# nreHieW/Eagle

Hardware: AMD Instinct MI355X
Metric: frames/sec end-to-end (detect+keypoint+homography) @1280x720 (higher is better)
Workload: dtype f32 (split: hi/lo binary16 pairs, 3 x fp16 MFMA per product, fp32 accumulate); detector (1.4 % of the FLOP): f32, exact v_mfma_f32_16x16x4_f32 chains

## Files before the change

eagle_amd/csrc/conv.hip:

```cpp
#include <algorithm>
#include <cmath>
#include <cstdlib>
#include <mutex>

#include "common.h"
#include "dmath.h"
#include "conv_internal.h"

namespace eagle {

static int f16_ps(int kc) { const int g = kc / 8; return kc * 2 + ((g % 2 == 0) ? 16 : 0); }
static int f16_ni(int ks, int kc) { return (ks * ks * (kc / 8) + 3) / 4; }

enum FormKind { GENERIC, WSTAT, ADIRECT };
enum StrideForm { S1, S2D, S2T, S1L };
enum WeightImage { W_F32, W_F16, W_F16_S2D, W_SPLIT, W_SPLIT_AD, W_SPLIT_S2D, W_SPLIT_M32 };
struct Form {
    int prec, variant, kind;
    int pw;
    int sform, rows, cols;
    int kc, nt, halo_bufs;
    int wimage;
    int grid_cap;
    ConvKernelGetter get;
};
static constexpr Form gen(int prec, int variant, int pw, int wimage, int kind = GENERIC) { return {prec, variant, kind, pw, S1, 0, 0, 0, 0, 0, wimage, 0, nullptr}; }
static constexpr Form ad(int prec, int variant, int sform, int rows, int cols, int nt, int halo_bufs, int wimage, ConvKernelGetter get, int grid_cap = 0)
{
    return {prec, variant, ADIRECT, 0, sform, rows, cols, prec == EAGLE_PREC_F16 ? 32 : 16, nt, halo_bufs, wimage, grid_cap, get};
}
static constexpr int F16 = EAGLE_PREC_F16, F32 = EAGLE_PREC_F32, F32S = EAGLE_PREC_F32S;
static constexpr Form g_forms[] = {
    gen(F32, 0, 4, W_F32), gen(F32, 3, 2, W_F32), gen(F32, 4, 1, W_F32),
    gen(F16, 0, 4, W_F16), gen(F16, 2, 4, W_F16), gen(F16, 3, 2, W_F16), gen(F16, 4, 1, W_F16), gen(F16, 6, 4, W_F16, WSTAT), gen(F16, 7, 2, W_F16, WSTAT),
    ad(F16, 8, S1, 4, 32, 12, 2, W_F16, conv_ad_kernel_s1_bn192), ad(F16, 9, S1, 8, 32, 6, 2, W_F16, conv_ad_kernel_s1_bn96),
    ad(F16, 10, S2D, 4, 32, 12, 2, W_F16_S2D, conv_ad_kernel_s2_bn192), ad(F16, 11, S2D, 8, 32, 6, 2, W_F16_S2D, conv_ad_kernel_s2_bn96),
    gen(F32S, 0, 4, W_SPLIT), gen(F32S, 3, 2, W_SPLIT), gen(F32S, 18, 6, W_SPLIT),
    ad(F32S, 8, S1, 4, 32, 12, 2, W_SPLIT_AD, conv_ad_split_kernel_bn192), ad(F32S, 9, S1, 8, 32, 6, 2, W_SPLIT_AD, conv_ad_split_kernel_bn96),
    ad(F32S, 10, S2D, 4, 32, 12, 2, W_SPLIT_S2D, conv_ad_split_kernel_s2_bn192), ad(F32S, 11, S2D, 8, 32, 6, 2, W_SPLIT_S2D, conv_ad_split_kernel_s2_bn96),
    ad(F32S, 12, S1, 8, 32, 3, 2, W_SPLIT_AD, conv_ad_split_kernel48), ad(F32S, 13, S1, 16, 32, 3, 1, W_SPLIT_AD, conv_ad_split_kernel48sb),
    ad(F32S, 19, S1, 16, 32, 3, 2, W_SPLIT_AD, conv_ad_split_kernel48ring, 256),
    ad(F32S, 14, S2T, 4, 32, 12, 1, W_SPLIT_AD, conv_ad_split_kernel_s2t_bn192), ad(F32S, 15, S2T, 4, 32, 6, 1, W_SPLIT_AD, conv_ad_split_kernel_s2t_bn96),
    ad(F32S, 21, S1, 4, 32, 12, 2, W_SPLIT_M32, conv_ad_split32_kernel_bn192), ad(F32S, 22, S1, 8, 32, 6, 2, W_SPLIT_M32, conv_ad_split32_kernel_bn96),
    ad(F32S, 23, S1, 2, 64, 12, 2, W_SPLIT_M32, conv_ad_split32_kernel_w64_bn192), ad(F32S, 24, S1, 4, 64, 6, 2, W_SPLIT_M32, conv_ad_split32_kernel_w64_bn96),
    ad(F32S, 27, S1L, 6, 30, 12, 2, W_SPLIT_M32, conv_ad_split32_kernel_lin30)};
static constexpr int LIN_PIXELS = 128;

static const Form* find_form(int precision, int variant)
{
    for (const Form& f : g_forms)
        if (f.prec == precision && f.variant == variant) return &f;
    return nullptr;
}
static const Form& form_of(int precision, const ConvConfig& c)
{
    const Form* f = find_form(precision, c.variant);
    if (!f) fail(EAGLE_E_NOKERNEL, "no conv kernel form: prec=%d variant=%d", precision, c.variant);
    return *f;
}
static int kind_of(int precision, const ConvConfig& c) { const Form* f = find_form(precision, c.variant); return f ? f->kind : -1; }

static size_t lds_bytes(int precision, const ConvConfig& c)
{
    const Form& f = form_of(precision, c);
    if (f.kind == ADIRECT) {
        int hpix, rec, strips;
        if (precision == EAGLE_PREC_F16) { hpix = f.sform == S2D ? (f.rows + 1) * 33 : (f.rows + 2) * 34; rec = 96; strips = 4 * 32 * 112; }
        else if (f.wimage == W_SPLIT_M32) { hpix = (f.rows + 2) * (f.cols + 2); rec = 80; strips = 4 * 32 * 128; }
        else { hpix = f.sform == S2T ? (2 * f.rows + 1) * 66 : (f.rows + 2) * 34; rec = 96; strips = 4 * 16 * 208; }
        const int slabs = ((hpix * rec + 1023) / 1024 + 3) / 4 * 4;
        return (size_t)f.halo_bufs * slabs * 1024 + strips;
    }
    const int th = 4 * f.pw / c.wx, tw = 16 * c.wx;
    const int hw = (tw - 1) * c.stride + c.ks, hh = (th - 1) * c.stride + c.ks;
    const int bn = c.nt * 16;
    if (precision == EAGLE_PREC_F16) {
        const size_t operands = (size_t)f16_ni(c.ks, c.kc) * 4 * bn * 16 + (size_t)hh * hw * f16_ps(c.kc);
        const size_t strips = (size_t)4 * f.pw * 16 * (bn * 2 + 16);
        return f.kind == WSTAT ? operands + strips + 16 : std::max(operands + 16, strips);
    }
    if (precision == EAGLE_PREC_F32S) {
        const size_t operands = (size_t)f16_ni(c.ks, c.kc) * 2 * 4 * bn * 16 + (size_t)hh * hw * f16_ps(2 * c.kc);
        const size_t strips = (size_t)4 * f.pw * 16 * (bn * 4 + 16);
        return std::max(operands + 16, strips);
    }
    return (size_t)c.ks * c.ks * (c.kc / 4) * 4 * bn * 4 + (size_t)hh * hw * (c.kc + 1) * 4;
}

size_t conv_lds_bytes(int precision, const ConvConfig& c) { return lds_bytes(precision, c); }
void conv_tile_shape(int precision, const ConvConfig& c, int* th, int* tw)
{
    const Form& f = form_of(precision, c);
    *th = f.kind == ADIRECT ? f.rows : 4 * f.pw / c.wx; *tw = f.kind == ADIRECT ? f.cols : 16 * c.wx;
}

int conv_tiles_per_frame(int precision, const ConvConfig& c, int ho, int wo)
{
    int th, tw;
    conv_tile_shape(precision, c, &th, &tw);
    if (form_of(precision, c).sform == S1L) return (ho * wo + LIN_PIXELS - 1) / LIN_PIXELS;
    return ((wo + tw - 1) / tw) * ((ho + th - 1) / th);
}

static const Inst* generic_inst(int precision, const ConvConfig& c)
{
    for (auto part : {conv_inst_part0, conv_inst_part1, conv_inst_part2, conv_inst_part3, conv_inst_split0, conv_inst_split1, conv_inst_split2}) {
        int n = 0;
        const Inst* t = part(&n);
        for (int k = 0; k < n; ++k)
            if (t[k].prec == precision && t[k].ks == c.ks && t[k].s == c.stride && t[k].kc == c.kc && t[k].nt == c.nt && t[k].variant == c.variant) return &t[k];
    }
    return nullptr;
}
bool conv_supported(int precision, const ConvConfig& c)
{
    const Form* f = find_form(precision, c.variant);
    if (f && f->kind == ADIRECT) return c.ks == 3 && c.stride == (f->sform == S1 || f->sform == S1L ? 1 : 2) && c.kc == f->kc && c.nt == f->nt;
    return f && generic_inst(precision, c);
}

struct Tuned { int ks, s, cin, cout, wo, kc, nt, wx, variant; };
static const Tuned g_tuned[] = {
#include "conv_tuned.inc"
    {0, 0, 0, 0, 0, 0, 0, 0, 0}};
static const Tuned g_tuned_f32[] = {
#include "conv_tuned_f32.inc"
    {0, 0, 0, 0, 0, 0, 0, 0, 0}};
static const Tuned g_tuned_split[] = {
#include "conv_tuned_split.inc"
    {0, 0, 0, 0, 0, 0, 0, 0, 0}};
static bool tuned_match(const Tuned& t, const ConvConfig& c, int wo, ConvConfig* q)
{
    if (t.ks != c.ks || t.s != c.stride || t.cin != c.cin || t.cout != c.cout_pad || t.wo != wo) return false;
    *q = c; q->kc = t.kc; q->nt = t.nt; q->wx = t.wx; q->variant = t.variant;
    return true;
}

static bool env_force(const char* name, int* a, int* b, int* c) { const char* f = getenv(name); return f && sscanf(f, "%d,%d,%d", a, b, c) == 3; }
static bool env_off(const char* name) { const char* e = getenv(name); return e && atoi(e) == 0; }

static const int g_nts[] = {6, 4, 3, 2, 1};
static ConvConfig with_ad(ConvConfig c, int kc, int v192, int v96)
{
    c.kc = kc;
    if (c.cout_pad % 192 == 0) { c.nt = 12; c.variant = v192; } else { c.nt = 6; c.variant = v96; }
    return c;
}

static ConvConfig choose_f32(ConvConfig c, int wo)
{
    ConvConfig q = c; q.kc = (c.cin < 16) ? 4 : 16;
    if (env_force("EAGLE_F32_FORCE", &q.nt, &q.wx, &q.variant) && (q.wx == 1 || q.wx == 2) && q.nt >= 1 && c.cout_pad % (16 * q.nt) == 0 &&
        conv_supported(EAGLE_PREC_F32, q) && lds_bytes(EAGLE_PREC_F32, q) <= 160 * 1024)
        return q;
    for (const Tuned& t : g_tuned_f32)
        if (tuned_match(t, c, wo, &q) && conv_supported(EAGLE_PREC_F32, q)) return q;
    c.nt = 1;
    for (int nt : g_nts)
        if (c.cout_pad % (16 * nt) == 0) { c.nt = nt; break; }
    c.kc = (c.cin < 16) ? 4 : 16;
    if (c.stride == 2 && c.ks == 3) {
        q = c; q.variant = 3;
        if (conv_supported(EAGLE_PREC_F32, q)) return q;
    }
    return c;
}

static ConvConfig choose_split(ConvConfig c, int wo, bool plain_epilogue)
{
    const int prec = EAGLE_PREC_F32S, cin = c.cin, cout = c.cout_pad;
    ConvConfig q = c;
    if (env_force("EAGLE_CONV_FORCE", &q.kc, &q.nt, &q.variant) && cin % q.kc == 0 && cout % (16 * q.nt) == 0 && conv_supported(prec, q) &&
        (form_of(prec, q).sform != S1L || (plain_epilogue && wo == form_of(prec, q).cols))) {
        if (form_of(prec, q).pw == 6) q.wx = 3;
        if (lds_bytes(prec, q) <= 160 * 1024) return q;
    }
    if (plain_epilogue && c.ks == 3 && c.stride == 2 && cin % 48 == 0 && cout % 96 == 0) return with_ad(c, 16, 14, 15);
    if (!env_off("EAGLE_CONV_M32") && plain_epilogue && c.ks == 3 && c.stride == 1 && cin % 16 == 0 && cout % 96 == 0) {
        q = with_ad(c, 16, 21, wo > 32 ? 24 : 22);
        if (q.variant == 21 && wo == 30) q.variant = 27;
        return q;
    }
    for (const Tuned& t : g_tuned_split)
        if (tuned_match(t, c, wo, &q)) {
            const Form* f = find_form(prec, q.variant);
            if (kind_of(prec, q) == ADIRECT && !(plain_epilogue && cin % (f->sform == S2D ? 16 : 48) == 0)) continue;
            if (conv_supported(prec, q) && lds_bytes(prec, q) <= 160 * 1024) return q;
        }
    if (plain_epilogue && c.ks == 3 && c.stride == 1 && cin % 48 == 0 && cout % 96 == 0) return with_ad(c, 16, 8, 9);
    static const int skcs[] = {32, 16, 8};
    long best = -1;
    c.nt = 1; c.kc = 8; c.variant = 0;
    for (int variant : {0, 3})
        for (int nt : g_nts) {
            if (cout % (16 * nt)) continue;
            for (int kc : skcs) {
                if (cin % kc) continue;
                ConvConfig t = c; t.nt = nt; t.kc = kc; t.variant = variant;
                if (!conv_supported(prec, t)) continue;
                if (lds_bytes(prec, t) > 80 * 1024) continue;
                const int pw = form_of(prec, t).pw;
                if (nt * pw > 12) continue;
                const long score = (long)nt * pw * 1000 + kc * 10 + (variant == 0 ? 1 : 0);
                if (score > best) { best = score; c.nt = nt; c.kc = kc; c.variant = variant; }
            }
        }
    return c;
}

static ConvConfig choose_f16(ConvConfig c, int wo, bool plain_epilogue, bool plain_one)
{
    const int prec = EAGLE_PREC_F16, cin = c.cin, cout = c.cout_pad;
    ConvConfig q = c;
    if (env_force("EAGLE_CONV_FORCE", &q.kc, &q.nt, &q.variant) && cin % q.kc == 0 && cout % (16 * q.nt) == 0 && conv_supported(prec, q) &&
        lds_bytes(prec, q) <= 160 * 1024 && (kind_of(prec, q) == WSTAT ? plain_one : kind_of(prec, q) == ADIRECT ? plain_epilogue : true))
        return q;
    if (plain_epilogue && c.ks == 3 && c.stride == 1 && cin % 32 == 0 && cout % 96 == 0) return with_ad(c, 32, 8, 9);
    if (plain_epilogue && c.ks == 3 && c.stride == 2 && cin % 8 == 0 && cin >= 32 && cout % 96 == 0) return with_ad(c, 32, 10, 11);
    for (const Tuned& t : g_tuned)
        if (tuned_match(t, c, wo, &q)) {
            if (kind_of(prec, q) == WSTAT && !plain_one) continue;
            if (conv_supported(prec, q) && lds_bytes(prec, q) <= 160 * 1024) return q;
        }
    static const int kcs[] = {64, 48, 32, 16, 8};
    long best = -1;
    c.nt = 1; c.kc = 8;
    for (int nt : g_nts) {
        if (cout % (16 * nt)) continue;
        for (int kc : kcs) {
            if (cin % kc) continue;
            ConvConfig t = c; t.nt = nt; t.kc = kc;
            if (!conv_supported(prec, t)) continue;
            if (lds_bytes(prec, t) > 80 * 1024) continue;
            const long score = (long)kc * nt * 1000 + kc;
            if (score > best) { best = score; c.nt = nt; c.kc = kc; }
        }
    }
    return c;
}

ConvConfig conv_choose(int precision, int ks, int stride, int cin_pad, int cout_pad, int wo, bool plain_epilogue, bool second_residual)
{
    ConvConfig c;
    c.ks = ks; c.stride = stride; c.cin = cin_pad; c.cout_pad = cout_pad;
    c.wx = (wo > 16) ? 2 : 1;
    if (precision == EAGLE_PREC_F32) return choose_f32(c, wo);
    if (precision == EAGLE_PREC_F32S) return choose_split(c, wo, plain_epilogue);
    return choose_f16(c, wo, plain_epilogue, plain_epilogue && !second_residual);
}

size_t conv_weight_elems(int precision, const ConvConfig& c)
{
    const int bn = c.nt * 16, nblk = c.cout_pad / bn, nch = c.cin / c.kc;
    switch (form_of(precision, c).wimage) {
    case W_F16_S2D: return (size_t)nblk * (4 * c.cin / 32) * 16 * bn * 8;
    case W_F16: return (size_t)nblk * nch * f16_ni(c.ks, c.kc) * 4 * bn * 8;
    case W_SPLIT_S2D: return (size_t)nblk * (4 * c.cin / 16) * 6 * 4 * bn * 8;
    case W_SPLIT_M32: return (size_t)nblk * (c.cin / 16) * 18 * (bn / 32) * 512;
    case W_SPLIT_AD: return (size_t)nblk * (c.cin / 16) * 14 * 4 * bn * 8;
    case W_SPLIT: return (size_t)nblk * nch * f16_ni(c.ks, c.kc) * 2 * 4 * bn * 8;
    default: return (size_t)nblk * nch * c.ks * c.ks * (c.kc / 4) * 4 * bn;
    }
}

void conv_tile_weights(int precision, const ConvConfig& c, const float* w, int cin_real, int cout_real, void* dst, float* descale)
{
    const int bn = c.nt * 16, nblk = c.cout_pad / bn, nch = c.cin / c.kc, taps = c.ks * c.ks, wimage = form_of(precision, c).wimage;
    auto W = [&](int tap, int ci, int co) -> float {
        return (ci < cin_real && co < cout_real) ? w[((size_t)tap * cin_real + ci) * cout_real + co] : 0.0f;
    };
    if (descale) *descale = 1.0f;
    if (precision == EAGLE_PREC_F32S) {
        float amax = 0.f;
        for (size_t k = 0; k < (size_t)taps * cin_real * cout_real; ++k) amax = std::max(amax, std::fabs(w[k]));
        int e = 0;
        if (amax > 0.f) (void)std::frexp(amax, &e);
        const int sw = 15 - e;
        const float scale = std::ldexp(1.0f, sw);
        if (descale) *descale = std::ldexp(1.0f, -(sw + 4));
        _Float16* d = (_Float16*)dst;
        if (wimage == W_SPLIT_S2D) {
            const int per_phase = c.cin / 16;
            for (int b = 0; b < nblk; ++b)
                for (int ch = 0; ch < 4 * per_phase; ++ch)
                    for (int k = 0; k < 6; ++k)
                        for (int qq = 0; qq < 4; ++qq)
                            for (int nn = 0; nn < bn; ++nn)
                                for (int j = 0; j < 8; ++j) {
                                    const int ph = ch / per_phase, c0 = (ch - ph * per_phase) * 16, ry = ph >> 1, rx = ph & 1;
                                    const int tp = k < 4 ? k : 2 * (k - 4) + (qq >> 1), tyy = tp >> 1, txx = tp & 1;
                                    const int ky = tyy == 0 ? (ry == 1 ? 0 : -1) : (ry == 0 ? 1 : 2), kx = txx == 0 ? (rx == 1 ? 0 : -1) : (rx == 0 ? 1 : 2);
                                    float v = 0.f;
                                    if (ky >= 0 && kx >= 0) v = W(ky * 3 + kx, c0 + (qq & 1) * 8 + j, b * bn + nn) * scale;
                                    const _Float16 hi = (_Float16)v;
                                    *d++ = k < 4 ? hi : (_Float16)(v - (float)hi);
                                }
            return;
        }
        if (wimage == W_SPLIT_M32) {
            for (int b = 0; b < nblk; ++b)
                for (int ch = 0; ch < c.cin / 16; ++ch)
                    for (int tap = 0; tap < 9; ++tap)
                        for (int part = 0; part < 2; ++part)
                            for (int mb = 0; mb < bn / 32; ++mb)
                                for (int l = 0; l < 64; ++l)
                                    for (int j = 0; j < 8; ++j) {
                                        const float v = W(tap, ch * 16 + (l >> 5) * 8 + j, b * bn + mb * 32 + (l & 31)) * scale;
                                        const _Float16 hi = (_Float16)v;
                                        *d++ = part == 0 ? hi : (_Float16)(v - (float)hi);
                                    }
            return;
        }
        if (wimage == W_SPLIT_AD) {
            for (int b = 0; b < nblk; ++b)
                for (int ch = 0; ch < c.cin / 16; ++ch)
                    for (int k = 0; k < 14; ++k)
                        for (int qq = 0; qq < 4; ++qq)
                            for (int nn = 0; nn < bn; ++nn)
                                for (int j = 0; j < 8; ++j) {
                                    const int tap = k < 9 ? k : 2 * (k - 9) + (qq >> 1);
                                    float v = 0.f;
                                    if (tap < 9) v = W(tap, ch * 16 + (qq & 1) * 8 + j, b * bn + nn) * scale;
                                    const _Float16 hi = (_Float16)v;
                                    *d++ = k < 9 ? hi : (_Float16)(v - (float)hi);
                                }
            return;
        }
        const int G = c.kc / 8, NGR = taps * G, NI = f16_ni(c.ks, c.kc);
        for (int b = 0; b < nblk; ++b)
            for (int ch = 0; ch < nch; ++ch)
                for (int i = 0; i < NI; ++i)
                    for (int part = 0; part < 2; ++part)
                        for (int qq = 0; qq < 4; ++qq)
// ... 156 lines not shown
```

eagle_amd/csrc/conv_ad_split32.hip:

```cpp
#include <algorithm>
#include <cstdlib>
#include <type_traits>

#include "common.h"
#include "dmath.h"
#include "conv_internal.h"

namespace eagle {

#include "conv_kernels.inc"
#include "conv_ad_split32.inc"

ConvKernel conv_ad_split32_kernel_bn192(int n_res, bool deep)
{
    static const ConvKernel fn[2][3] = {
        {conv_split_ad32_kernel<2, 2, 0>, conv_split_ad32_kernel<2, 2, 1>, conv_split_ad32_kernel<2, 2, 2>},
        {conv_split_ad32_kernel<2, 2, 0, 6>, conv_split_ad32_kernel<2, 2, 1, 6>, conv_split_ad32_kernel<2, 2, 2, 6>}};
    return fn[deep ? 1 : 0][res_slot(n_res)];
}

ConvKernel conv_ad_split32_kernel_bn96(int n_res, bool deep)
{
    static const ConvKernel fn[2][3] = {
        {conv_split_ad32_kernel<1, 4, 0>, conv_split_ad32_kernel<1, 4, 1>, conv_split_ad32_kernel<1, 4, 2>},
        {conv_split_ad32_kernel<1, 4, 0, 6>, conv_split_ad32_kernel<1, 4, 1, 6>, conv_split_ad32_kernel<1, 4, 2, 6>}};
    return fn[deep ? 1 : 0][res_slot(n_res)];
}

ConvKernel conv_ad_split32_kernel_w64_bn192(int n_res, bool deep)
{
    static const ConvKernel fn[2][3] = {
        {conv_split_ad32_kernel<2, 2, 0, 3, 2>, conv_split_ad32_kernel<2, 2, 1, 3, 2>, conv_split_ad32_kernel<2, 2, 2, 3, 2>},
        {conv_split_ad32_kernel<2, 2, 0, 6, 2>, conv_split_ad32_kernel<2, 2, 1, 6, 2>, conv_split_ad32_kernel<2, 2, 2, 6, 2>}};
    return fn[deep ? 1 : 0][res_slot(n_res)];
}

ConvKernel conv_ad_split32_kernel_w64_bn96(int n_res, bool deep)
{
    static const ConvKernel fn[2][3] = {
        {conv_split_ad32_kernel<1, 4, 0, 3, 2>, conv_split_ad32_kernel<1, 4, 1, 3, 2>, conv_split_ad32_kernel<1, 4, 2, 3, 2>},
        {conv_split_ad32_kernel<1, 4, 0, 6, 2>, conv_split_ad32_kernel<1, 4, 1, 6, 2>, conv_split_ad32_kernel<1, 4, 2, 6, 2>}};
    return fn[deep ? 1 : 0][res_slot(n_res)];
}

ConvKernel conv_ad_split32_kernel_lin30(int n_res, bool deep)
{
    static const ConvKernel fn[2][3] = {
        {conv_split_ad32_kernel<2, 2, 0, 3, 1, 30>, conv_split_ad32_kernel<2, 2, 1, 3, 1, 30>, conv_split_ad32_kernel<2, 2, 2, 3, 1, 30>},
        {conv_split_ad32_kernel<2, 2, 0, 6, 1, 30>, conv_split_ad32_kernel<2, 2, 1, 6, 1, 30>, conv_split_ad32_kernel<2, 2, 2, 6, 1, 30>}};
    return fn[deep ? 1 : 0][res_slot(n_res)];
}

}
```

eagle_amd/csrc/conv_ad_split32.inc:

```
#ifndef EAGLE_CONV_AD_SPLIT32_INC
#define EAGLE_CONV_AD_SPLIT32_INC
#ifndef EAGLE_ABL_M32
#define EAGLE_ABL_M32 0
#endif
#ifndef EAGLE_M32_RES_NT
#define EAGLE_M32_RES_NT 1
#endif
#ifndef EAGLE_M32_SAUX
#define EAGLE_M32_SAUX (EAGLE_STORE_NT * 2 + EAGLE_M32_RES_NT * 4)
#endif
using f32x16 = __attribute__((ext_vector_type(16))) float;
#if EAGLE_ABL_M32 == 1 || EAGLE_ABL_M32 == 6
__device__ __forceinline__ f32x16 abl_m32_xor(const half8& a_, const half8& b_, f32x16 c_)
{
    const u32x4 ua = __builtin_bit_cast(u32x4, a_), ub = __builtin_bit_cast(u32x4, b_);
    c_[0] = __builtin_bit_cast(float, __builtin_bit_cast(unsigned, c_[0]) ^ ua[0] ^ ub[3]);
    return c_;
}
#define EAGLE_MFMA_M32(A_, B_, C_) abl_m32_xor(A_, B_, C_)
#else
#define EAGLE_MFMA_M32(A_, B_, C_) __builtin_amdgcn_mfma_f32_32x32x16_f16(A_, B_, C_, 0, 0, 0)
#endif
__device__ __forceinline__ void split_store4x(char* dhi, char* dlo, float v0, float v1, float v2, float v3)
{
    const float s0 = __builtin_amdgcn_fmed3f(v0 * SPLIT_SX, -65504.0f, 65504.0f), s1 = __builtin_amdgcn_fmed3f(v1 * SPLIT_SX, -65504.0f, 65504.0f),
                s2 = __builtin_amdgcn_fmed3f(v2 * SPLIT_SX, -65504.0f, 65504.0f), s3 = __builtin_amdgcn_fmed3f(v3 * SPLIT_SX, -65504.0f, 65504.0f);
    const half4 hi = {(_Float16)s0, (_Float16)s1, (_Float16)s2, (_Float16)s3};
    const half4 lo = {(_Float16)(s0 - (float)hi[0]), (_Float16)(s1 - (float)hi[1]), (_Float16)(s2 - (float)hi[2]), (_Float16)(s3 - (float)hi[3])};
    *(half4*)dhi = hi; *(half4*)dlo = lo;
}
template <int CQ, int PG, int RES, int RING = 3, int NRH = 1, int MAPW = 0>
__global__ __launch_bounds__(256, 2) void conv_split_ad32_kernel(ConvArgs a)
{
    static_assert(CQ * PG == 4, "four waves per workgroup");
    constexpr bool LIN = MAPW != 0;
    static_assert(!LIN || (CQ == 2 && PG == 2 && NRH == 1 && MAPW == 30), "linear tiling: the BN = 192 form on the 30-column map");
    static_assert(NRH == 1 || NRH == 2, "the wave's two pixel blocks: one above the other (1) or side by side (2)");
    static_assert(18 % RING == 0 && RING >= 3, "the weight ring holds a divisor of the 18 steps of a chunk");
    using rsrc_t = __amdgpu_buffer_rsrc_t;
    constexpr unsigned OOB = 0x80000000u;
    constexpr int MB = 3, NR = 2, NRV = NR / NRH, NW = 4, BN = CQ * 96, TH = NRV * PG, TW = 32 * NRH;
    constexpr int KSTEP = (BN / 32) * 1024;
    constexpr int PS = 80, SPC = 18, AHEAD = RING - 1;
    constexpr int LROWS = LIN ? (128 - 2) / (LIN ? MAPW : 1) + 2 : 0;
    constexpr int HW_ = LIN ? MAPW + 2 : TW + 2, HPIX = (LIN ? LROWS + 2 : TH + 2) * HW_;
    constexpr int HSLABS = ((HPIX * PS + 1023) / 1024 + NW - 1) / NW * NW, HB = HSLABS * 1024, HK = HSLABS / NW;
    constexpr int RS = 32 * 4, STRIP = 32 * RS;
    extern __shared__ __attribute__((aligned(16))) char smem[];
    char* const Hb = smem;
    char* const strip = smem + 2 * HB + (threadIdx.x >> 6) * STRIP;
    const int tid = threadIdx.x, lane = tid & 63, wave = __builtin_amdgcn_readfirstlane(tid >> 6);
    const int cq = wave % CQ, pg = wave / CQ, kh = lane >> 5, lx = lane & 31;
    const int gy = a.gy, nitems = a.tiles_x * a.tiles_y * a.N * gy, nwg = gridDim.x;
    int item0, item_end;
    {
        const int b = blockIdx.x, xcd = b & 7, k = b >> 3;
        const int wgs_here = (nwg + 7 - xcd) >> 3;
        const int qn = nitems >> 3, rn = nitems & 7;
        const int x0 = xcd < rn ? xcd * (qn + 1) : rn * (qn + 1) + (xcd - rn) * qn;
        const int xc = qn + (xcd < rn ? 1 : 0);
        item0 = x0 + (int)((long)xc * k / wgs_here);
        item_end = x0 + (int)((long)xc * (k + 1) / wgs_here);
    }
    if (item0 >= item_end) return;
    const int nloc = item_end - item0, nch = a.nchunks, GC = nloc * nch;
    const rsrc_t xrs = __builtin_amdgcn_make_buffer_rsrc((void*)a.x, 0, 0x7FFFFFFF, 0x00020000);
    const rsrc_t wrs = __builtin_amdgcn_make_buffer_rsrc((void*)a.w, 0, 0x7FFFFFFF, 0x00020000);
    const rsrc_t rrs = __builtin_amdgcn_make_buffer_rsrc((void*)a.r1, 0, 0x7FFFFFFF, 0x00020000);
    const rsrc_t rrs2 = __builtin_amdgcn_make_buffer_rsrc((void*)a.r2, 0, 0x7FFFFFFF, 0x00020000);
    const rsrc_t yrs = __builtin_amdgcn_make_buffer_rsrc((void*)a.y, 0, 0x7FFFFFFF, 0x00020000);
    constexpr bool RECOMP = HK > 6;
    const int e0 = wave * 64 + lane;
    int hpk[RECOMP ? 1 : HK];
    if constexpr (!RECOMP) {
#pragma unroll
        for (int k = 0; k < HK; ++k) {
            const int e = e0 + NW * 64 * k;
            const int pix = e / 5, slot = e - pix * 5;
            const int hy = pix / HW_, hx = pix - hy * HW_;
            hpk[k] = (pix < HPIX && slot < 4) ? (hy | (hx << 8) | (((slot & 1) * 2 + (slot >> 1)) << 16)) : -1;
        }
    }
    const int bbase = ((pg * NRV) * HW_ + lx) * PS + kh * 16;
    const unsigned wlane = (unsigned)((cq * MB * 64 + lane) * 16);

    auto decode = [&](int item, int& n, int& ty, int& tx, int& nb) {
        int t = item / gy; nb = item - t * gy;
        tx = t % a.tiles_x; t /= a.tiles_x;
        ty = t % a.tiles_y; n = t / a.tiles_y;
    };
    int h_g = 0, h_ch = 0, h_item = item0;
    int h_iy0, h_ix0, h_gb;
    auto halo_origin = [&](int item) {
        int n, ty, tx, nb; decode(item, n, ty, tx, nb);
        if constexpr (LIN) { h_iy0 = (tx * 128) / MAPW - 1; h_ix0 = -1; }
        else { h_iy0 = ty * TH - 1; h_ix0 = tx * TW - 1; }
        h_gb = (((n * a.H + h_iy0) * a.W + h_ix0) * a.xcs + a.xoff) * 2;
    };
    halo_origin(h_item);
    auto issue_h_slab = [&](int k) {
        char* dst = Hb + (h_g & 1) * HB;
        const unsigned so = (EAGLE_ABL_M32 == 8) ? 0u : (unsigned)(h_ch * 32) * 2u;
        int hy, hx, unit; bool live;
        if constexpr (RECOMP) {
            int e = e0 + NW * 64 * k;
            asm volatile("" : "+v"(e));
            const int pix = (int)(((unsigned)e * 52429u) >> 18), slot = e - pix * 5;
            hy = HW_ == 34 ? (int)(((unsigned)pix * 1928u) >> 16) : (int)(((unsigned)pix * 993u) >> 16); hx = pix - hy * HW_;
            unit = (slot & 1) * 2 + (slot >> 1);
            live = pix < HPIX && slot < 4;
        } else {
            hy = hpk[k] & 0xFF; hx = (hpk[k] >> 8) & 0xFF; unit = (hpk[k] >> 16) & 7; live = hpk[k] >= 0;
        }
        const int iy = h_iy0 + hy, ix = h_ix0 + hx;
        const unsigned off = !(live && (unsigned)iy < (unsigned)a.H && (unsigned)ix < (unsigned)a.W) ? OOB
                             : (unsigned)(h_gb + ((hy * a.W + hx) * a.xcs + unit * 8) * 2);
        __builtin_amdgcn_raw_ptr_buffer_load_lds(xrs, (__attribute__((address_space(3))) void*)(dst + (wave + NW * k) * 1024), 16,
                                                 ((EAGLE_ABL_M32 == 3 || EAGLE_ABL_M32 == 6 || EAGLE_ABL_M32 == 7) && h_g > 0) ? OOB : off, so, 0, 0);
    };
    auto advance_h = [&]() {
        if (h_g + 1 >= GC) return;
        ++h_g;
        if (++h_ch == nch) { h_ch = 0; ++h_item; halo_origin(h_item); }
    };
    auto issue_h = [&]() {
#pragma unroll
        for (int k = 0; k < HK; ++k) issue_h_slab(k);
        advance_h();
    };
    issue_h();
    int gc = 0;
    for (int item = item0; item < item_end; ++item) {
        int n, ty, tx, nb; decode(item, n, ty, tx, nb);
        const int oy0 = ty * TH, ox0 = tx * TW;
        const int L0 = tx * 128, npix = a.H * a.W;
        int bbl[LIN ? NR : 1];
        if constexpr (LIN) {
            const int yf = L0 / MAPW;
#pragma unroll
            for (int p = 0; p < NR; ++p) {
                const int L = min(L0 + (pg * NR + p) * 32 + lx, npix - 1), y = L / MAPW, x = L - y * MAPW;
                bbl[p] = ((y - yf) * HW_ + x) * PS + kh * 16;
            }
        }
        f32x16 acc[MB][NR];
#pragma unroll
        for (int i = 0; i < MB; ++i)
#pragma unroll
            for (int p = 0; p < NR; ++p)
#pragma unroll
                for (int r = 0; r < 16; ++r) acc[i][p][r] = 0.f;
        u32x4 A[RING][MB];
        unsigned wsrc = (unsigned)(nb * nch * SPC) * (unsigned)KSTEP;
        const unsigned wend = wsrc + (unsigned)(nch * SPC) * (unsigned)KSTEP;
        bool abl_a_done = false;
        auto load_a = [&](int slot) {
            const unsigned so = wsrc < wend ? wsrc : wend - KSTEP;
#pragma unroll
            for (int mb = 0; mb < MB; ++mb)
                if (!((EAGLE_ABL_M32 == 2 || EAGLE_ABL_M32 == 6 || EAGLE_ABL_M32 == 7) && abl_a_done)) A[slot][mb] = __builtin_amdgcn_raw_buffer_load_b128(wrs, wlane + mb * 1024, so, 0);
            wsrc += KSTEP;
        };
#pragma unroll
        for (int s = 0; s < AHEAD; ++s) load_a(s);
        abl_a_done = true;
        for (int ch = 0; ch < nch; ++ch, ++gc) {
            if constexpr (AHEAD * MB == 6) asm volatile("s_waitcnt vmcnt(6)" ::: "memory");
            else asm volatile("s_waitcnt vmcnt(15)" ::: "memory");
            static_assert(AHEAD * MB == 6 || AHEAD * MB == 15, "vmcnt literal");
            __builtin_amdgcn_s_barrier();
            issue_h();
            const char* hb = Hb + (gc & 1) * HB + bbase;
            const char* hbl[LIN ? NR : 1];
            if constexpr (LIN) {
#pragma unroll
                for (int p = 0; p < NR; ++p) hbl[p] = Hb + (gc & 1) * HB + bbl[p];
            }
            half8 Bh[2][NR], Bl[2][NR];
            auto read_b = [&](int slot, int tap) {
                const int ky = tap / 3, kx = tap - ky * 3;
#pragma unroll
                for (int p = 0; p < NR; ++p) {
                    if constexpr (LIN) {
                        Bh[slot][p] = *(const half8*)(hbl[p] + (ky * HW_ + kx) * PS);
                        Bl[slot][p] = *(const half8*)(hbl[p] + (ky * HW_ + kx) * PS + 32);
                    } else {
                        Bh[slot][p] = *(const half8*)(hb + ((p / NRH + ky) * HW_ + (p % NRH) * 32 + kx) * PS);
                        Bl[slot][p] = *(const half8*)(hb + ((p / NRH + ky) * HW_ + (p % NRH) * 32 + kx) * PS + 32);
                    }
                }
            };
            read_b(0, 0);
#pragma unroll
            for (int t = 0; t < 9; ++t) {
                const int bs = (EAGLE_ABL_M32 == 4 || EAGLE_ABL_M32 == 6) ? 0 : (t & 1);
                load_a((2 * t + AHEAD) % RING);
                if (t + 1 < 9 && !(EAGLE_ABL_M32 == 4 || EAGLE_ABL_M32 == 6)) read_b((t + 1) & 1, t + 1);
#pragma unroll
                for (int p = 0; p < NR; ++p)
#pragma unroll
                    for (int mb = 0; mb < MB; ++mb) acc[mb][p] = EAGLE_MFMA_M32((half8)A[(2 * t) % RING][mb], Bh[bs][p], acc[mb][p]);
#pragma unroll
                for (int p = 0; p < NR; ++p)
#pragma unroll
                    for (int mb = 0; mb < MB; ++mb) acc[mb][p] = EAGLE_MFMA_M32((half8)A[(2 * t) % RING][mb], Bl[bs][p], acc[mb][p]);
                __builtin_amdgcn_sched_barrier(0);
                load_a((2 * t + 1 + AHEAD) % RING);
#pragma unroll
                for (int p = 0; p < NR; ++p)
#pragma unroll
                    for (int mb = 0; mb < MB; ++mb) acc[mb][p] = EAGLE_MFMA_M32((half8)A[(2 * t + 1) % RING][mb], Bh[bs][p], acc[mb][p]);
                __builtin_amdgcn_sched_barrier(0);
            }
        }
        const int co0 = nb * BN + cq * 96;
        __builtin_amdgcn_sched_barrier(0);
        const float ds = a.descale;
        int pstrip[4], ppx[4];
#pragma unroll
        for (int i = 0; i < 4; ++i) {
            const int e = i * 64 + lane, px = e >> 3, u = e & 7;
            pstrip[i] = px * RS + ((u ^ (px & 7)) * 16);
            ppx[i] = px | (u << 8);
        }
        auto piece_off = [&](int pass, int i, int cs, int off) -> unsigned {
            const int row = pass / MB, mb = pass - row * MB;
            if constexpr (LIN) {
                const int L = L0 + (pg * NR + row) * 32 + (ppx[i] & 0xFF), u = ppx[i] >> 8;
                return L < npix ? (unsigned)(((n * npix + L) * cs + off + (co0 + mb * 32) * 2 + u * 8) * 2) : OOB;
            }
            const int oy = oy0 + pg * NRV + row / NRH, ox2 = ox0 + (row % NRH) * 32 + (ppx[i] & 0xFF), u = ppx[i] >> 8;
            return (oy < a.Ho && ox2 < a.Wo) ? (unsigned)((((n * a.Ho + oy) * a.Wo + ox2) * cs + off + (co0 + mb * 32) * 2 + u * 8) * 2) : OOB;
        };
        float vmax = 0.0f;
        constexpr int NPASS = NR * MB, PB = (RES == 2 && NRH == 2) ? 2 : (RES == 2 || (RES == 1 && NRH == 2)) ? 3 : 6;
        u32x4 rres[RES >= 1 ? PB : 1][4], rres2[RES >= 2 ? PB : 1][4];
        char* const sp = strip + lx * RS + kh * 8;
        const int sw = (lx & 7) * 16;
        auto run_hi = [&](int j) -> char* { return sp + ((j * 32) ^ sw); };
        auto run_lo = [&](int j) -> char* { return sp + ((j * 32 + 16) ^ sw); };
#pragma unroll
        for (int pb0 = 0; pb0 < NPASS; pb0 += PB) {
            if (RES >= 1) {
#pragma unroll
                for (int h2 = 0; h2 < PB; ++h2)
#pragma unroll
                    for (int i = 0; i < 4; ++i) rres[h2][i] = __builtin_amdgcn_raw_buffer_load_b128(rrs, piece_off(pb0 + h2, i, a.r1cs, a.r1off), 0, (EAGLE_M32_SAUX & 4) ? 2 : 0);
            }
            if (RES >= 2) {
#pragma unroll
                for (int h2 = 0; h2 < PB; ++h2)
#pragma unroll
                    for (int i = 0; i < 4; ++i) rres2[h2][i] = __builtin_amdgcn_raw_buffer_load_b128(rrs2, piece_off(pb0 + h2, i, a.r2cs, a.r2off), 0, (EAGLE_M32_SAUX & 4) ? 2 : 0);
            }
#pragma unroll
            for (int h2 = 0; h2 < PB; ++h2) {
                const int pass = pb0 + h2, row = pass / MB, mb = pass - row * MB;
                if (RES >= 1) {
#pragma unroll
                    for (int i = 0; i < 4; ++i) *(u32x4*)(strip + pstrip[i]) = rres[h2][i];
                }
                float v[4][4];
#pragma unroll
                for (int j = 0; j < 4; ++j) {
                    const float4 bv = *(const float4*)(a.bias + co0 + mb * 32 + j * 8 + kh * 4);
                    v[j][0] = acc[mb][row][j * 4 + 0] * ds + bv.x; v[j][1] = acc[mb][row][j * 4 + 1] * ds + bv.y;
                    v[j][2] = acc[mb][row][j * 4 + 2] * ds + bv.z; v[j][3] = acc[mb][row][j * 4 + 3] * ds + bv.w;
                    if (RES >= 1) {
                        const half4 rh = *(const half4*)run_hi(j), rl = *(const half4*)run_lo(j);
#pragma unroll
                        for (int r = 0; r < 4; ++r) v[j][r] = ((float)rh[r] + (float)rl[r]) * SPLIT_RX + v[j][r];
                    }
                }
                if (RES >= 2) {
#pragma unroll
                    for (int i = 0; i < 4; ++i) *(u32x4*)(strip + pstrip[i]) = rres2[h2][i];
#pragma unroll
                    for (int j = 0; j < 4; ++j) {
                        const half4 rh = *(const half4*)run_hi(j), rl = *(const half4*)run_lo(j);
#pragma unroll
                        for (int r = 0; r < 4; ++r) v[j][r] = v[j][r] + ((float)rh[r] + (float)rl[r]) * SPLIT_RX;
                    }
                }
#pragma unroll
                for (int j = 0; j < 4; ++j) {
                    if (a.post_act == 1) {
#pragma unroll
                        for (int r = 0; r < 4; ++r) v[j][r] = v[j][r] > 0.f ? v[j][r] : 0.f;
                    }
                    split_store4x(run_hi(j), run_lo(j), v[j][0], v[j][1], v[j][2], v[j][3]);
                    vmax = split_absmax4(vmax, v[j][0], v[j][1], v[j][2], v[j][3]);
                }
#pragma unroll
                for (int i = 0; i < 4; ++i)
                    __builtin_amdgcn_raw_buffer_store_b128(*(const u32x4*)(strip + pstrip[i]), yrs, (EAGLE_ABL_M32 >= 5 && EAGLE_ABL_M32 <= 7) ? OOB : piece_off(pass, i, a.ycs, a.yoff), 0, EAGLE_M32_SAUX & 3);
            }
        }
        split_report(a.sat, n, vmax);
    }
}

#endif
```

eagle_amd/csrc/conv_internal.h:

```cpp
#pragma once
#include "common.h"

namespace eagle {

using half8 = __attribute__((ext_vector_type(8))) _Float16;
using half4 = __attribute__((ext_vector_type(4))) _Float16;
using f32x4 = __attribute__((ext_vector_type(4))) float;
using u32x4 = __attribute__((ext_vector_type(4))) unsigned int;
using u32x2 = __attribute__((ext_vector_type(2))) unsigned int;

struct ConvArgs {
    const void* x; int xcs, xoff; int N, H, W;
    const void* w; const float* bias;
    void* y; int ycs, yoff; int Ho, Wo;
    const void* r1; int r1cs, r1off;
    const void* r2; int r2cs, r2off;
    int pre_act, post_act, out_f32;
    int wx, tiles_x, tiles_y, nchunks;
    int gy;
    int stack;
    int xcd;
    ArgmaxPart* am;
    int am_cs;
    float descale;
    const void* zeros;
    void* trash;
    unsigned* sat;
};

struct BneckArgs {
    const void* x; int xcs, xoff; int N, H, W, nch1;
    const void *w1, *w2, *w3; const float *b1, *b2, *b3; float ds1, ds2, ds3;
    const void* r; int rcs, roff;
    void* y; int ycs, yoff;
    int tiles_x, tiles_y;
    unsigned* sat;
    unsigned long long* dbg;
};

typedef void (*ConvKernel)(ConvArgs);
struct Inst { int prec, ks, s, kc, nt, variant; ConvKernel fn; };
const Inst* conv_inst_part0(int* n); const Inst* conv_inst_part1(int* n); const Inst* conv_inst_part2(int* n); const Inst* conv_inst_part3(int* n);
const Inst* conv_inst_split0(int* n); const Inst* conv_inst_split1(int* n); const Inst* conv_inst_split2(int* n);
inline int res_slot(int n_res) { return n_res < 0 ? 0 : n_res > 2 ? 2 : n_res; }
typedef ConvKernel (*ConvKernelGetter)(int n_res, bool deep);
ConvKernel conv_ad_kernel_s1_bn192(int n_res, bool deep);
ConvKernel conv_ad_kernel_s1_bn96(int n_res, bool deep);
ConvKernel conv_ad_kernel_s2_bn192(int n_res, bool deep);
ConvKernel conv_ad_kernel_s2_bn96(int n_res, bool deep);
ConvKernel conv_ad_split_kernel_bn192(int n_res, bool deep);
ConvKernel conv_ad_split_kernel_bn96(int n_res, bool deep);
ConvKernel conv_ad_split_kernel_s2_bn192(int n_res, bool deep);
ConvKernel conv_ad_split_kernel_s2_bn96(int n_res, bool deep);
ConvKernel conv_ad_split_kernel_s2t_bn192(int n_res, bool deep);
ConvKernel conv_ad_split_kernel_s2t_bn96(int n_res, bool deep);
ConvKernel conv_ad_split_kernel48(int n_res, bool deep);
ConvKernel conv_ad_split_kernel48sb(int n_res, bool deep);
ConvKernel conv_ad_split_kernel48ring(int n_res, bool deep);
ConvKernel conv_ad_split32_kernel_bn192(int n_res, bool deep);
ConvKernel conv_ad_split32_kernel_bn96(int n_res, bool deep);
ConvKernel conv_ad_split32_kernel_w64_bn192(int n_res, bool deep);
ConvKernel conv_ad_split32_kernel_w64_bn96(int n_res, bool deep);
ConvKernel conv_ad_split32_kernel_lin30(int n_res, bool deep);

}
```

Before: 846.4.

## Add linear-tiled split32 conv form for 60-column feature maps

Extends the linear pixel tiling, where each 128-pixel item spans whole rows, from the 30-column map to the 60-column map. It adds variant 28, which uses a shared halo indexing helper to compute compact halo records from the item's origin row and column, and selects it when the output width is 60. The aim is to avoid the wasted padded pixels and halo loads of the rectangular 32- or 64-wide tiles on a 60-wide map. In exchange it adds per-item halo index recomputation and a different residual prefetch depth.

```diff
diff --git a/eagle_amd/csrc/conv.hip b/eagle_amd/csrc/conv.hip
--- a/eagle_amd/csrc/conv.hip
+++ b/eagle_amd/csrc/conv.hip
@@ -6,6 +6,7 @@
 #include "common.h"
 #include "dmath.h"
 #include "conv_internal.h"
+#include "conv_lin_index.h"
 
 namespace eagle {
 
@@ -43,8 +44,8 @@
     ad(F32S, 14, S2T, 4, 32, 12, 1, W_SPLIT_AD, conv_ad_split_kernel_s2t_bn192), ad(F32S, 15, S2T, 4, 32, 6, 1, W_SPLIT_AD, conv_ad_split_kernel_s2t_bn96),
     ad(F32S, 21, S1, 4, 32, 12, 2, W_SPLIT_M32, conv_ad_split32_kernel_bn192), ad(F32S, 22, S1, 8, 32, 6, 2, W_SPLIT_M32, conv_ad_split32_kernel_bn96),
     ad(F32S, 23, S1, 2, 64, 12, 2, W_SPLIT_M32, conv_ad_split32_kernel_w64_bn192), ad(F32S, 24, S1, 4, 64, 6, 2, W_SPLIT_M32, conv_ad_split32_kernel_w64_bn96),
-    ad(F32S, 27, S1L, 6, 30, 12, 2, W_SPLIT_M32, conv_ad_split32_kernel_lin30)};
-static constexpr int LIN_PIXELS = 128;
+    ad(F32S, 27, S1L, 6, 30, 12, 2, W_SPLIT_M32, conv_ad_split32_kernel_lin30), ad(F32S, 28, S1L, 4, 60, 12, 2, W_SPLIT_M32, conv_ad_split32_kernel_lin60)};
+static constexpr int LIN_PIXELS = lin::LIN_ITEM;
 
 static const Form* find_form(int precision, int variant)
 {
@@ -66,7 +67,7 @@
     if (f.kind == ADIRECT) {
         int hpix, rec, strips;
         if (precision == EAGLE_PREC_F16) { hpix = f.sform == S2D ? (f.rows + 1) * 33 : (f.rows + 2) * 34; rec = 96; strips = 4 * 32 * 112; }
-        else if (f.wimage == W_SPLIT_M32) { hpix = (f.rows + 2) * (f.cols + 2); rec = 80; strips = 4 * 32 * 128; }
+        else if (f.wimage == W_SPLIT_M32) { hpix = f.sform == S1L ? lin::halo_records(f.cols) : (f.rows + 2) * (f.cols + 2); rec = 80; strips = 4 * 32 * 128; }
         else { hpix = f.sform == S2T ? (2 * f.rows + 1) * 66 : (f.rows + 2) * 34; rec = 96; strips = 4 * 16 * 208; }
         const int slabs = ((hpix * rec + 1023) / 1024 + 3) / 4 * 4;
         return (size_t)f.halo_bufs * slabs * 1024 + strips;
@@ -179,6 +180,7 @@
     if (!env_off("EAGLE_CONV_M32") && plain_epilogue && c.ks == 3 && c.stride == 1 && cin % 16 == 0 && cout % 96 == 0) {
         q = with_ad(c, 16, 21, wo > 32 ? 24 : 22);
         if (q.variant == 21 && wo == 30) q.variant = 27;
+        if (q.variant == 21 && wo == 60) q.variant = 28;
         return q;
     }
     for (const Tuned& t : g_tuned_split)
diff --git a/eagle_amd/csrc/conv_ad_split32.hip b/eagle_amd/csrc/conv_ad_split32.hip
--- a/eagle_amd/csrc/conv_ad_split32.hip
+++ b/eagle_amd/csrc/conv_ad_split32.hip
@@ -5,6 +5,7 @@
 #include "common.h"
 #include "dmath.h"
 #include "conv_internal.h"
+#include "conv_lin_index.h"
 
 namespace eagle {
 
@@ -51,4 +52,12 @@
     return fn[deep ? 1 : 0][res_slot(n_res)];
 }
 
+ConvKernel conv_ad_split32_kernel_lin60(int n_res, bool deep)
+{
+    static const ConvKernel fn[2][3] = {
+        {conv_split_ad32_kernel<2, 2, 0, 3, 1, 60>, conv_split_ad32_kernel<2, 2, 1, 3, 1, 60>, conv_split_ad32_kernel<2, 2, 2, 3, 1, 60>},
+        {conv_split_ad32_kernel<2, 2, 0, 6, 1, 60>, conv_split_ad32_kernel<2, 2, 1, 6, 1, 60>, conv_split_ad32_kernel<2, 2, 2, 6, 1, 60>}};
+    return fn[deep ? 1 : 0][res_slot(n_res)];
 }
+
+}
diff --git a/eagle_amd/csrc/conv_ad_split32.inc b/eagle_amd/csrc/conv_ad_split32.inc
--- a/eagle_amd/csrc/conv_ad_split32.inc
+++ b/eagle_amd/csrc/conv_ad_split32.inc
@@ -34,7 +34,7 @@
 {
     static_assert(CQ * PG == 4, "four waves per workgroup");
     constexpr bool LIN = MAPW != 0;
-    static_assert(!LIN || (CQ == 2 && PG == 2 && NRH == 1 && MAPW == 30), "linear tiling: the BN = 192 form on the 30-column map");
+    static_assert(!LIN || (CQ == 2 && PG == 2 && NRH == 1 && (MAPW == 30 || MAPW == 60)), "linear tiling: the BN = 192 form on the 30- and 60-column maps");
     static_assert(NRH == 1 || NRH == 2, "the wave's two pixel blocks: one above the other (1) or side by side (2)");
     static_assert(18 % RING == 0 && RING >= 3, "the weight ring holds a divisor of the 18 steps of a chunk");
     using rsrc_t = __amdgpu_buffer_rsrc_t;
@@ -42,8 +42,8 @@
     constexpr int MB = 3, NR = 2, NRV = NR / NRH, NW = 4, BN = CQ * 96, TH = NRV * PG, TW = 32 * NRH;
     constexpr int KSTEP = (BN / 32) * 1024;
     constexpr int PS = 80, SPC = 18, AHEAD = RING - 1;
-    constexpr int LROWS = LIN ? (128 - 2) / (LIN ? MAPW : 1) + 2 : 0;
-    constexpr int HW_ = LIN ? MAPW + 2 : TW + 2, HPIX = (LIN ? LROWS + 2 : TH + 2) * HW_;
+    static_assert(!LIN || lin::LIN_ITEM == PG * NR * 32, "a linear item is the workgroup's PG x NR blocks of 32 pixels");
+    constexpr int HW_ = LIN ? lin::halo_w(LIN ? MAPW : 1) : TW + 2, HPIX = LIN ? lin::halo_records(LIN ? MAPW : 1) : (TH + 2) * HW_;
     constexpr int HSLABS = ((HPIX * PS + 1023) / 1024 + NW - 1) / NW * NW, HB = HSLABS * 1024, HK = HSLABS / NW;
     constexpr int RS = 32 * 4, STRIP = 32 * RS;
     extern __shared__ __attribute__((aligned(16))) char smem[];
@@ -71,8 +71,9 @@
     const rsrc_t yrs = __builtin_amdgcn_make_buffer_rsrc((void*)a.y, 0, 0x7FFFFFFF, 0x00020000);
     constexpr bool RECOMP = HK > 6;
     const int e0 = wave * 64 + lane;
+    static_assert(!LIN || !RECOMP, "the linear forms hold the decomposition of the item being requested");
     int hpk[RECOMP ? 1 : HK];
-    if constexpr (!RECOMP) {
+    if constexpr (!RECOMP && !LIN) {
 #pragma unroll
         for (int k = 0; k < HK; ++k) {
             const int e = e0 + NW * 64 * k;
@@ -93,8 +94,17 @@
     int h_iy0, h_ix0, h_gb;
     auto halo_origin = [&](int item) {
         int n, ty, tx, nb; decode(item, n, ty, tx, nb);
-        if constexpr (LIN) { h_iy0 = (tx * 128) / MAPW - 1; h_ix0 = -1; }
-        else { h_iy0 = ty * TH - 1; h_ix0 = tx * TW - 1; }
+        if constexpr (LIN) {
+            const lin::Origin o = lin::item_origin(tx, MAPW);
+            h_iy0 = o.yf - 1; h_ix0 = -1;
+#pragma unroll
+            for (int k = 0; k < HK; ++k) {
+                const int e = e0 + NW * 64 * k;
+                const int pix = (int)(((unsigned)e * 52429u) >> 18), slot = e - pix * 5;
+                const int hy = lin::record_row(pix, o.xf, MAPW), hx = lin::record_col(pix, o.xf, MAPW);
+                hpk[k] = (pix < HPIX && slot < 4) ? (hy | (hx << 8) | (((slot & 1) * 2 + (slot >> 1)) << 16)) : -1;
+            }
+        } else { h_iy0 = ty * TH - 1; h_ix0 = tx * TW - 1; }
         h_gb = (((n * a.H + h_iy0) * a.W + h_ix0) * a.xcs + a.xoff) * 2;
     };
     halo_origin(h_item);
@@ -133,14 +143,14 @@
     for (int item = item0; item < item_end; ++item) {
         int n, ty, tx, nb; decode(item, n, ty, tx, nb);
         const int oy0 = ty * TH, ox0 = tx * TW;
-        const int L0 = tx * 128, npix = a.H * a.W;
+        const int L0 = tx * lin::LIN_ITEM, npix = a.H * a.W;
         int bbl[LIN ? NR : 1];
         if constexpr (LIN) {
-            const int yf = L0 / MAPW;
+            const lin::Origin o = lin::item_origin(tx, MAPW);
 #pragma unroll
             for (int p = 0; p < NR; ++p) {
                 const int L = min(L0 + (pg * NR + p) * 32 + lx, npix - 1), y = L / MAPW, x = L - y * MAPW;
-                bbl[p] = ((y - yf) * HW_ + x) * PS + kh * 16;
+                bbl[p] = lin::fragment_base(y, x, o, MAPW) * PS + kh * 16;
             }
         }
         f32x16 acc[MB][NR];
@@ -216,10 +226,13 @@
         const int co0 = nb * BN + cq * 96;
         __builtin_amdgcn_sched_barrier(0);
         const float ds = a.descale;
+        int elane = lane;
+        if constexpr (MAPW == 60) asm volatile("" : "+v"(elane));
+        const int ekh = elane >> 5, elx = elane & 31;
         int pstrip[4], ppx[4];
 #pragma unroll
         for (int i = 0; i < 4; ++i) {
-            const int e = i * 64 + lane, px = e >> 3, u = e & 7;
+            const int e = i * 64 + elane, px = e >> 3, u = e & 7;
             pstrip[i] = px * RS + ((u ^ (px & 7)) * 16);
             ppx[i] = px | (u << 8);
         }
@@ -233,10 +246,10 @@
             return (oy < a.Ho && ox2 < a.Wo) ? (unsigned)((((n * a.Ho + oy) * a.Wo + ox2) * cs + off + (co0 + mb * 32) * 2 + u * 8) * 2) : OOB;
         };
         float vmax = 0.0f;
-        constexpr int NPASS = NR * MB, PB = (RES == 2 && NRH == 2) ? 2 : (RES == 2 || (RES == 1 && NRH == 2)) ? 3 : 6;
+        constexpr int NPASS = NR * MB, PB = (RES == 2 && NRH == 2) ? 2 : (RES == 2 || (RES == 1 && (NRH == 2 || MAPW == 60))) ? 3 : 6;
         u32x4 rres[RES >= 1 ? PB : 1][4], rres2[RES >= 2 ? PB : 1][4];
-        char* const sp = strip + lx * RS + kh * 8;
-        const int sw = (lx & 7) * 16;
+        char* const sp = strip + elx * RS + ekh * 8;
+        const int sw = (elx & 7) * 16;
         auto run_hi = [&](int j) -> char* { return sp + ((j * 32) ^ sw); };
         auto run_lo = [&](int j) -> char* { return sp + ((j * 32 + 16) ^ sw); };
 #pragma unroll
@@ -263,7 +276,7 @@
                 float v[4][4];
 #pragma unroll
                 for (int j = 0; j < 4; ++j) {
-                    const float4 bv = *(const float4*)(a.bias + co0 + mb * 32 + j * 8 + kh * 4);
+                    const float4 bv = *(const float4*)(a.bias + co0 + mb * 32 + j * 8 + ekh * 4);
                     v[j][0] = acc[mb][row][j * 4 + 0] * ds + bv.x; v[j][1] = acc[mb][row][j * 4 + 1] * ds + bv.y;
                     v[j][2] = acc[mb][row][j * 4 + 2] * ds + bv.z; v[j][3] = acc[mb][row][j * 4 + 3] * ds + bv.w;
                     if (RES >= 1) {
diff --git a/eagle_amd/csrc/conv_internal.h b/eagle_amd/csrc/conv_internal.h
--- a/eagle_amd/csrc/conv_internal.h
+++ b/eagle_amd/csrc/conv_internal.h
@@ -62,5 +62,6 @@
 ConvKernel conv_ad_split32_kernel_w64_bn192(int n_res, bool deep);
 ConvKernel conv_ad_split32_kernel_w64_bn96(int n_res, bool deep);
 ConvKernel conv_ad_split32_kernel_lin30(int n_res, bool deep);
+ConvKernel conv_ad_split32_kernel_lin60(int n_res, bool deep);
 
 }
diff --git a/eagle_amd/csrc/conv_lin_index.h b/eagle_amd/csrc/conv_lin_index.h
--- /dev/null
+++ b/eagle_amd/csrc/conv_lin_index.h
@@ -0,0 +1,73 @@
+#ifndef EAGLE_CONV_LIN_INDEX_H
+#define EAGLE_CONV_LIN_INDEX_H
+
+#if defined(__HIPCC__) || defined(__CUDACC__)
+#define EAGLE_LIN_HD __host__ __device__
+#else
+#define EAGLE_LIN_HD
+#endif
+
+namespace eagle {
+namespace lin {
+
+constexpr int LIN_ITEM = 128;
+
+EAGLE_LIN_HD constexpr int halo_w(int W) { return W + 2; }
+EAGLE_LIN_HD constexpr int max_crossings(int W) { return (W - 1 + LIN_ITEM - 1) / W; }
+EAGLE_LIN_HD constexpr int halo_records(int W) { return 2 * W + LIN_ITEM + 6 + 2 * max_crossings(W); }
+EAGLE_LIN_HD constexpr int items_per_frame(int H, int W) { return (H * W + LIN_ITEM - 1) / LIN_ITEM; }
+
+struct Origin { int yf, xf; };
+EAGLE_LIN_HD constexpr Origin item_origin(int t, int W) { const int L0 = t * LIN_ITEM, yf = L0 / W; return {yf, L0 - yf * W}; }
+
+struct Pixel { int iy, ix; };
+EAGLE_LIN_HD constexpr int record_row(int r, int xf, int W) { return (xf + r) / halo_w(W); }
+EAGLE_LIN_HD constexpr int record_col(int r, int xf, int W) { return (xf + r) - record_row(r, xf, W) * halo_w(W); }
+EAGLE_LIN_HD constexpr Pixel record_pixel(int r, Origin o, int W) { return {o.yf - 1 + record_row(r, o.xf, W), record_col(r, o.xf, W) - 1}; }
+
+EAGLE_LIN_HD constexpr int fragment_base(int y, int x, Origin o, int W) { return (y - o.yf) * halo_w(W) + x - o.xf; }
+EAGLE_LIN_HD constexpr int tap_offset(int ky, int kx, int W) { return ky * halo_w(W) + kx; }
+
+constexpr bool map_is_covered(int H, int W)
+{
+    const int npix = H * W, hpix = halo_records(W);
+    for (int t = 0; t < items_per_frame(H, W); ++t) {
+        const Origin o = item_origin(t, W);
+        if (o.yf * W + o.xf != t * LIN_ITEM || o.xf < 0 || o.xf >= W) return false;
+        for (int l = 0; l < LIN_ITEM; ++l) {
+            const int L = t * LIN_ITEM + l < npix ? t * LIN_ITEM + l : npix - 1, y = L / W, x = L - y * W;
+            for (int ky = 0; ky < 3; ++ky)
+                for (int kx = 0; kx < 3; ++kx) {
+                    const int r = fragment_base(y, x, o, W) + tap_offset(ky, kx, W);
+                    if (r < 0 || r >= hpix) return false;
+                    const Pixel p = record_pixel(r, o, W);
+                    if (p.iy != y - 1 + ky || p.ix != x - 1 + kx) return false;
+                    if (p.ix < -1 || p.ix > W || p.iy < -1 || p.iy > H) return false;
+                }
+        }
+    }
+    return true;
+}
+constexpr bool halo_is_tight(int H, int W)
+{
+    const int npix = H * W;
+    for (int t = 0; t < items_per_frame(H, W); ++t) {
+        const int Ll = t * LIN_ITEM + LIN_ITEM - 1;
+        if (Ll >= npix) continue;
+        const Origin o = item_origin(t, W);
+        if (fragment_base(Ll / W, Ll % W, o, W) + tap_offset(2, 2, W) == halo_records(W) - 1) return true;
+    }
+    return false;
+}
+
+static_assert(halo_records(30) == 204 && halo_records(60) == 260, "halo records per item");
+static_assert(map_is_covered(17, 30) && map_is_covered(34, 60), "HRNet's maps");
+static_assert(map_is_covered(1, 30) && map_is_covered(2, 30) && map_is_covered(3, 30) && map_is_covered(5, 30) && map_is_covered(9, 30) && map_is_covered(32, 30), "30 columns, odd heights");
+static_assert(map_is_covered(1, 60) && map_is_covered(2, 60) && map_is_covered(3, 60) && map_is_covered(5, 60) && map_is_covered(9, 60) && map_is_covered(32, 60), "60 columns, odd heights");
+static_assert(map_is_covered(7, 60) && map_is_covered(7, 30) && map_is_covered(70, 30), "further heights");
+static_assert(halo_is_tight(32, 30) && halo_is_tight(34, 60), "the halo has no spare record");
+
+}
+}
+
+#endif
```

New measurement: 853.8, median of 6. About the same (+0.9%).
